# muyangyi/SimSeg

Hardware: AMD Instinct MI355X
Metric: image-text pairs/sec (train) + seg images/sec (eval), ViT-B (higher is better)
Workload: dtype fp16

## Files before the change

simseg_amd/csrc/gemm.hip:

```cpp
#include "common.h"
#include <type_traits>

#ifdef SS_GEMM_ABLATE
#define SS_ABL(v) (p.stagger == (v))
#else
#define SS_ABL(v) false
#endif

namespace {

constexpr int BM = 128, BN = 128, NTHREADS = 256;
constexpr int MC_PITCH = 320;
template <int KB> struct Geo {
    static constexpr int KC_PITCH = KB + 16;
    static constexpr int NCH = KB / 16;
    static constexpr int LOADS = 128 * NCH / NTHREADS;
    static constexpr int KROWS = KB / 2;
    static constexpr int TILE_BYTES = (128 * KC_PITCH > KROWS * MC_PITCH) ? 128 * KC_PITCH : KROWS * MC_PITCH;
    static constexpr int KSTEPS = KB / 32;
};

struct GemmParams {
    const void* A; const void* B; void* C;
    int M, N, K;
// ... 1059 lines not shown
__device__ __forceinline__ const GemmParams& pp_params(const GemmParams& arg, const GemmParams&) { return arg; }
__device__ __forceinline__ const GemmParams& pp_params(const WgradGroupParams&, const GemmParams& own) { return own; }

template <typename TO, bool TA, bool TB, int PP_LEAD = 4, int PRIO = 1, int BIG = 0, int EK = 1, bool GROUPED = false, bool ATOMIC_DIRECT = false>
__global__ __launch_bounds__(512, 2) void gemm_pp_kernel(typename std::conditional<GROUPED, WgradGroupParams, GemmParams>::type arg) {
    extern __shared__ __attribute__((aligned(16))) char lds[];
    GemmParams own;
    int gkz = 0, gt = 0;
    if constexpr (GROUPED) {
        const int gq = xcd_remap(blockIdx.x, gridDim.x);
        if (gq >= arg.first[arg.n]) return;
        int i = 0;
#pragma unroll
        for (int j = 1; j < WG_MAX; ++j)
            if (j < arg.n && gq >= arg.first[j]) i = j;
        const WgradProblem& w = arg.prob[i];
        own = GemmParams{};
        own.A = w.dy; own.B = w.x; own.C = w.dw;
        own.M = w.out; own.N = w.in; own.K = arg.rows;
        own.lda = w.ld_dy; own.ldb = w.ld_x; own.ldc = w.ld_dw;
        own.alpha = 1.0f;
        own.accumulate = 1;
        own.ksplit = arg.ksplit; own.nsplit = arg.nsplit;
        own.dbg_trace = arg.dbg_trace;
        const int gtiles = (w.out >> 8) * (w.in >> 8);
        const int r = gq - arg.first[i];
        gkz = r / gtiles;
        gt = r - gkz * gtiles;
    }
    const GemmParams& p = pp_params(arg, own);
    const int tid = threadIdx.x, lane = tid & 63, wave = __builtin_amdgcn_readfirstlane(tid >> 6);
    const int grp = wave >> 2, wn = wave & 3;
    const int tiles_n = (p.N + 255) / 256;
    const int tiles = tiles_n * ((p.M + 255) / 256);
    const int q = xcd_remap(blockIdx.x, gridDim.x);
    const int kz = GROUPED ? gkz : q / tiles, t = GROUPED ? gt : q - kz * tiles;
    const int m0 = (t / tiles_n) * 256, n0 = (t % tiles_n) * 256;
    const int nk = p.K / 64;
    const int kt0 = kz * p.ksplit;
    const int ntile = min(nk, kt0 + p.ksplit) - kt0;
    const int stot = 4 * ntile;
    const char* Ab = static_cast<const char*>(p.A) + (TA ? (long)kt0 * 64 * p.lda * 2 : (long)kt0 * 128);
    const char* Bb = static_cast<const char*>(p.B) + (TB ? (long)kt0 * 64 * p.ldb * 2 : (long)kt0 * 128);
    const long astep = TA ? 64 * p.lda * 2 : 128, bstep = TB ? 64 * p.ldb * 2 : 128;
    long dA = 0, dB = 0;
    bool pf_ok = false;
    if (BIG && p.pf_next && p.nsplit == 1) {
        const int nb8 = (int)gridDim.x >> 3, rr8 = (int)gridDim.x & 7, xx = (int)blockIdx.x & 7, jj = (int)blockIdx.x >> 3;
        if (jj + 32 < nb8 + (xx < rr8 ? 1 : 0)) {
            const int tn_ = t + 32;
            const int m1 = (tn_ / tiles_n) * 256, n1 = (tn_ % tiles_n) * 256;
            if (m0 + 256 <= p.M && n0 + 256 <= p.N && m1 + 256 <= p.M && n1 + 256 <= p.N) {
                pf_ok = true;
                dA = TA ? (long)(m1 - m0) * 2 : (long)(m1 - m0) * p.lda * 2;
                dB = TB ? (long)(n1 - n0) * 2 : (long)(n1 - n0) * p.ldb * 2;
            }
        }
    }
    unsigned offA[2][2], offB[2][2];
#pragma unroll
    for (int h = 0; h < 2; ++h)
#pragma unroll
        for (int i = 0; i < 2; ++i) {
            offA[h][i] = pp_src_off<TA>(wave * 2 + i, lane, m0 + h * 128, p.M, p.lda);
            offB[h][i] = pp_src_off<TB>(wave * 2 + i, lane, n0 + h * 128, p.N, p.ldb);
            asm volatile("" : "+v"(offA[h][i]), "+v"(offB[h][i]));
        }
    const unsigned lds0 = (unsigned)(unsigned long)(__attribute__((address_space(3))) char*)lds;
    PPFrag<TA, 2> fra;
    PPFrag<TB, 1> frb;
    fra.init(0, grp * 64, lane);
    frb.init(PP_BREG, wn * 32, lane);

    f32x16 acc[4][2];
    {
        const f32x16 zero = {0.f, 0.f, 0.f, 0.f, 0.f, 0.f, 0.f, 0.f, 0.f, 0.f, 0.f, 0.f, 0.f, 0.f, 0.f, 0.f};
#pragma unroll
        for (int i = 0; i < 4; ++i)
#pragma unroll
            for (int j = 0; j < 2; ++j) acc[i][j] = zero;
    }
#define PP_STAGE(H_, KIND)                                                                                            \
    {                                                                                                                 \
        const int h_ = (H_);                                                                                          \
        const bool live_ = h_ < stot;                                                                                 \
        const int kt_ = live_ ? (h_ >> 2) : (pf_ok ? ((h_ - stot) >> 2) : ntile - 1);                                 \
        const unsigned dst_ = lds0 + (live_ ? (((KIND) & 1) ? 0 : PP_BREG) + (((h_ >> 2) & 1) * 2 + ((KIND) >> 1)) * PP_HALF : PP_DUMMY) + \
                              wave * 2048;                                                                            \
        const char* sb_ = ((KIND) & 1) ? Ab + kt_ * astep + (live_ ? 0 : dA) : Bb + kt_ * bstep + (live_ ? 0 : dB);   \
        pp_glds16(((KIND) & 1) ? offA[(KIND) >> 1][0] : offB[(KIND) >> 1][0], sb_, dst_);                             \
        pp_glds16(((KIND) & 1) ? offA[(KIND) >> 1][1] : offB[(KIND) >> 1][1], sb_, dst_ + 1024);                      \
    }
    u32x4 fa[8], fb0[4], fb1[4];
#define PP_READ_A(PAR, HALF)                                                                       \
    _Pragma("unroll") for (int i_ = 0; i_ < 2; ++i_)                                               \
        _Pragma("unroll") for (int kk_ = 0; kk_ < 4; ++kk_) fa[i_ * 4 + kk_] = fra.read(lds, ((PAR) * 2 + (HALF)) * PP_HALF, i_, kk_);
#define PP_READ_B(FB, PAR, HALF) \
    _Pragma("unroll") for (int kk_ = 0; kk_ < 4; ++kk_) FB[kk_] = frb.read(lds, ((PAR) * 2 + (HALF)) * PP_HALF, 0, kk_);
#define PP_CLUSTER(RH, CH, FB)                                                                       \
    if (PRIO == 1) __builtin_amdgcn_s_setprio(1);                                                    \
    _Pragma("unroll") for (int kk_ = 0; kk_ < 4; ++kk_)                                              \
        _Pragma("unroll") for (int i_ = 0; i_ < 2; ++i_) mma<bf16_t>(acc[2 * (RH) + i_][CH], fa[i_ * 4 + kk_], FB[kk_]); \
    if (PRIO == 1) __builtin_amdgcn_s_setprio(0);

    if (p.stagger > 0 && blockIdx.x < 256) {
        const unsigned long long until = wall_clock64() + (unsigned long long)(((blockIdx.x >> 3) & 3) * p.stagger);
        while (wall_clock64() < until) __builtin_amdgcn_s_sleep(8);
    }
    unsigned long long tr0 = 0, tr1 = 0, tr2 = 0;
    if (p.dbg_trace) tr0 = wall_clock64();
    if constexpr (BIG) {
        PP_STAGE(0, 0) PP_STAGE(1, 1) PP_STAGE(2, 2) PP_STAGE(3, 3) PP_STAGE(4, 0) PP_STAGE(5, 1) PP_STAGE(6, 2)
        wait_vm<8>();
        __builtin_amdgcn_s_barrier();
        __builtin_amdgcn_sched_barrier(0);
        if (grp == 1) __builtin_amdgcn_s_barrier();
        if (p.dbg_trace) tr1 = wall_clock64();
#define PP_BIGPHASE(READS, STAGES, RH, CA, FA_, CB, FB_)                                       \
    {                                                                                          \
        READS                                                                                  \
        STAGES                                                                                 \
        wait_vm<8>();                                                                          \
        __builtin_amdgcn_sched_barrier(0);                                                     \
        __builtin_amdgcn_s_barrier();                                                          \
        asm volatile("s_waitcnt lgkmcnt(0)" ::: "memory");                                     \
        __builtin_amdgcn_sched_barrier(0);                                                     \
        PP_CLUSTER(RH, CA, FA_)                                                                \
        PP_CLUSTER(RH, CB, FB_)                                                                \
        asm volatile("" : "+v"(acc[2 * (RH)][0]), "+v"(acc[2 * (RH) + 1][0]), "+v"(acc[2 * (RH)][1]), "+v"(acc[2 * (RH) + 1][1])); \
        __builtin_amdgcn_sched_barrier(0);                                                     \
        __builtin_amdgcn_s_barrier();                                                          \
        __builtin_amdgcn_sched_barrier(0);                                                     \
    }
        for (int tt = 0; tt < ntile; ++tt) {
            PP_BIGPHASE(PP_READ_B(fb0, 0, 0) PP_READ_A(0, 0) PP_READ_B(fb1, 0, 1), PP_STAGE(4 * tt + 7, 3), 0, 0, fb0, 1, fb1)
            frb.toggle(2 * PP_HALF);
            PP_BIGPHASE(PP_READ_A(0, 1), PP_STAGE(4 * tt + 8, 0) PP_STAGE(4 * tt + 9, 1) PP_STAGE(4 * tt + 10, 2), 1, 1, fb1, 0, fb0)
            fra.toggle(2 * PP_HALF);
        }
#undef PP_BIGPHASE
    } else {
    PP_STAGE(0, 0) PP_STAGE(1, 1) PP_STAGE(2, 2) PP_STAGE(3, 3)
    if (PP_LEAD >= 4) PP_STAGE(4, 0)
    if (PP_LEAD >= 5) PP_STAGE(5, 1)
    wait_vm<2 * (PP_LEAD - 1)>();
    if (PRIO == 2 && grp == 1) __builtin_amdgcn_s_setprio(1);
    __builtin_amdgcn_s_barrier();
    __builtin_amdgcn_sched_barrier(0);
    PP_READ_B(fb0, 0, 0)
    if (grp == 1) __builtin_amdgcn_s_barrier();
    if (p.dbg_trace) tr1 = wall_clock64();

#define PP_PHASE(M_, Q, READS, RH, CH, FB)                                                     \
    {                                                                                          \
        READS                                                                                  \
        PP_STAGE((M_) + 1 + PP_LEAD, ((Q) + 1 + PP_LEAD) & 3)                                  \
        wait_vm<2 * (PP_LEAD - 1)>();                                                          \
        __builtin_amdgcn_sched_barrier(0);                                                     \
        __builtin_amdgcn_s_barrier();                                                          \
        asm volatile("s_waitcnt lgkmcnt(0)" ::: "memory");                                     \
        __builtin_amdgcn_sched_barrier(0);                                                     \
        PP_CLUSTER(RH, CH, FB)                                                                 \
        __builtin_amdgcn_sched_barrier(0);                                                     \
        __builtin_amdgcn_s_barrier();                                                          \
        __builtin_amdgcn_sched_barrier(0);                                                     \
    }
    for (int tt = 0; tt < ntile; ++tt) {
        PP_PHASE(4 * tt + 0, 0, PP_READ_A(0, 0), 0, 0, fb0)
        PP_PHASE(4 * tt + 1, 1, PP_READ_B(fb1, 0, 1), 0, 1, fb1)
        PP_PHASE(4 * tt + 2, 2, PP_READ_A(0, 1), 1, 1, fb1)
        frb.toggle(2 * PP_HALF);
        PP_PHASE(4 * tt + 3, 3, PP_READ_B(fb1, 0, 0), 1, 0, fb0)
        fra.toggle(2 * PP_HALF);
#pragma unroll
        for (int kk = 0; kk < 4; ++kk) fb0[kk] = fb1[kk];
    }
#undef PP_PHASE
    }
#undef PP_STAGE
#undef PP_READ_A
#undef PP_READ_B
#undef PP_CLUSTER
    if (!pf_ok) wait_vm<0>();
    if (grp == 0) __builtin_amdgcn_s_barrier();
    if (p.dbg_trace) tr2 = wall_clock64();

    const bool atomic = p.nsplit > 1;
    const bool vec_ok = epilogue_vec_ok(p, sizeof(TO));
    float* wlds = reinterpret_cast<float*>(lds) + wave * EP_WAVE_FLOATS;
    float cs[8] = {0.f, 0.f, 0.f, 0.f, 0.f, 0.f, 0.f, 0.f};
    const int c0 = n0 + wn * 32, c1 = c0 + 128;
    if constexpr (sizeof(TO) == 2) {
        const bool fastep = !atomic && vec_ok && !p.residual && !p.rowscale && p.row_group == 0 && !p.drop_thresh && !p.dbg_skip_epilogue &&
                            (p.act == 0 || p.act == 1 || (p.act == 3 && (!p.aux_blocked || (EK == 2 && p.aux_blocked == 1) || (EK == 4 && p.aux_blocked == 2))) ||
                             (((EK == 1 && !p.aux_blocked) || (EK == 3 && p.aux_blocked == 1) || (EK == 5 && p.aux_blocked == 2)) && p.act == 4 && p.aux)) && (p.act == 4 || !p.colsum) &&
                            m0 + 256 <= p.M && n0 + 256 <= p.N;
        if (fastep) {
            pp_epilogue_bf16<EK>(p, acc, reinterpret_cast<char*>(wlds), m0, c0, c1, grp, lane);
            if (pf_ok) wait_vm<16>();
            if (p.dbg_trace && tid == 0) {
                const unsigned long long tr3 = wall_clock64();
                asm volatile("s_waitcnt vmcnt(0)" ::: "memory");
                unsigned long long* d = p.dbg_trace + (long)blockIdx.x * 5;
                d[0] = tr0; d[1] = tr1; d[2] = tr2; d[3] = wall_clock64(); d[4] = tr3;
            }
            return;
        }
    }
    if constexpr (sizeof(TO) == 4) {
        const bool direct = !atomic && !p.rowscale && !p.aux && p.act == 0 && p.row_group == 0 && !p.colsum && !p.accumulate &&
                            !p.dbg_skip_epilogue && m0 + 256 <= p.M && n0 + 256 <= p.N;
        if (direct) {
            pp_epilogue_f32_direct(p, acc, m0, c0, c1, grp, lane);
            if (pf_ok) wait_vm<63>();
            if (p.dbg_trace && tid == 0) {
                const unsigned long long tr3 = wall_clock64();
                asm volatile("s_waitcnt vmcnt(0)" ::: "memory");
                unsigned long long* d = p.dbg_trace + (long)blockIdx.x * 5;
                d[0] = tr0; d[1] = tr1; d[2] = tr2; d[3] = wall_clock64(); d[4] = tr3;
            }
            return;
        }
    }
    if constexpr (ATOMIC_DIRECT && sizeof(TO) == 4) {
        if (atomic && !p.dbg_skip_epilogue && m0 + 256 <= p.M && n0 + 256 <= p.N) {
            pp_epilogue_atomic_direct(p, acc, m0, c0, c1, grp, lane);
            if (p.dbg_trace && tid == 0) {
                const unsigned long long tr3 = wall_clock64();
                asm volatile("s_waitcnt vmcnt(0)" ::: "memory");
                unsigned long long* d = p.dbg_trace + (long)blockIdx.x * 5;
                d[0] = tr0; d[1] = tr1; d[2] = tr2; d[3] = wall_clock64(); d[4] = tr3;
            }
            return;
        }
    }
#pragma unroll 1
    for (int i = 0; i < 4; ++i) {
        f32x16 l = acc[0][0], r = acc[0][1];
#pragma unroll
        for (int ii = 1; ii < 4; ++ii)
            if (ii == i) { l = acc[ii][0]; r = acc[ii][1]; }
        if (p.dbg_trace && tid == 0) p.dbg_trace[(long)gridDim.x * 5 + (long)blockIdx.x * 4 + i] = wall_clock64();
        epilogue_block<TO>(p, l, r, wlds, m0 + (i >> 1) * 128 + grp * 64 + (i & 1) * 32, c0, c1, lane, atomic, vec_ok, cs);
    }
    flush_colsum(p, cs, c0, c1, lane);
    if (pf_ok) wait_vm<0>();
    if (p.dbg_trace && tid == 0) {
        const unsigned long long tr3 = wall_clock64();
        asm volatile("s_waitcnt vmcnt(0)" ::: "memory");
        unsigned long long* d = p.dbg_trace + (long)blockIdx.x * 5;
        d[0] = tr0; d[1] = tr1; d[2] = tr2; d[3] = wall_clock64(); d[4] = tr3;
    }
}

template <typename TO, bool TA, bool TB, int LEAD = 4, int PRIO = 1, int BIG = 0, int EK = 1>
int launch_pp(const GemmParams& p, int splitk, hipStream_t stream) {
    constexpr int SMEM = 9 * PP_HALF;
    static bool configured = false;
    auto kern = gemm_pp_kernel<TO, TA, TB, LEAD, PRIO, BIG, EK>;
    if (!configured) {
        hipError_t e = hipFuncSetAttribute(reinterpret_cast<const void*>(kern), hipFuncAttributeMaxDynamicSharedMemorySize, SMEM);
        if (e != hipSuccess) return simseg_set_error("simseg_gemm: cannot reserve %d bytes of LDS: %s", SMEM, hipGetErrorString(e));
        configured = true;
    }
    const int tiles = ((p.M + 255) / 256) * ((p.N + 255) / 256);
    const int nk = p.K / 64;
    GemmParams q = p;
    if (splitk < 1) splitk = 1;
    if (splitk > nk) splitk = nk;
    q.ksplit = (nk + splitk - 1) / splitk;
    const int z = (nk + q.ksplit - 1) / q.ksplit;
    q.nsplit = z;
    hipLaunchKernelGGL(kern, dim3(tiles * z, 1, 1), dim3(512), SMEM, stream, q);
    SS_LAUNCH_CHECK("simseg_gemm(ping-pong)");
    return 0;
}

template <bool TRANS>
__device__ __forceinline__ unsigned pp2_lane_off(int piece, int lane, long ld) {
    if (!TRANS) {
        const int r = piece * 8 + (lane >> 3);
        const int c = (lane & 7) ^ kc_swz<64>(r);
        return (unsigned)((long)r * ld * 2 + c * 16);
    } else {
        const int kr = piece * 4 + (lane >> 4);
        const int c = (lane & 15) ^ ((kr & 3) << 2);
        return (unsigned)((long)kr * ld * 2 + c * 16);
    }
}

struct PP2Item { int m0, n0, ntile; const char* a0; const char* b0; };

template <bool TA, bool TB>
__device__ __forceinline__ PP2Item pp2_item(const GemmParams& p, int t, int tiles_n) {
    PP2Item it;
    it.m0 = (t / tiles_n) << 8;
    it.n0 = (t % tiles_n) << 8;
    it.ntile = p.K >> 6;
    it.a0 = static_cast<const char*>(p.A) + (TA ? (long)it.m0 * 2 : (long)it.m0 * p.lda * 2);
    it.b0 = static_cast<const char*>(p.B) + (TB ? (long)it.n0 * 2 : (long)it.n0 * p.ldb * 2);
    return it;
}

template <typename TO, bool TA, bool TB, int SCHED = 0, int EK = 1>
__global__ __launch_bounds__(512, 2) void gemm_pp2_kernel(GemmParams p) {
    extern __shared__ __attribute__((aligned(16))) char lds[];
    const int tid = threadIdx.x, lane = tid & 63, wave = __builtin_amdgcn_readfirstlane(tid >> 6);
    const int grp = wave >> 2, wn = wave & 3;
    const int tiles_n = p.N >> 8;
    const int total = tiles_n * (p.M >> 8);
    const int stride = (int)gridDim.x >> 3;
    const int x = blockIdx.x & 7;
    int ord = blockIdx.x >> 3;
    const int cq = total >> 3, cr = total & 7;
    const int cnt = cq + (x < cr ? 1 : 0);
    const int base = x < cr ? x * (cq + 1) : cr * (cq + 1) + (x - cr) * cq;
    if (ord >= cnt) return;
    const long astep = TA ? 64 * p.lda * 2 : 128, bstep = TB ? 64 * p.ldb * 2 : 128;
    const long ahalf = TA ? 256 : 128 * p.lda * 2, bhalf = TB ? 256 : 128 * p.ldb * 2;
    unsigned offA[2], offB[2];
#pragma unroll
    for (int i = 0; i < 2; ++i) {
        offA[i] = pp2_lane_off<TA>(wave * 2 + i, lane, p.lda);
        offB[i] = pp2_lane_off<TB>(wave * 2 + i, lane, p.ldb);
        asm volatile("" : "+v"(offA[i]), "+v"(offB[i]));
    }
    const unsigned lds0 = (unsigned)(unsigned long)(__attribute__((address_space(3))) char*)lds;
    PPFrag<TA, 2> fra;
    PPFrag<TB, 1> frb;
    fra.init(0, grp * 64, lane);
    frb.init(PP_BREG, wn * 32, lane);

    PP2Item cur = pp2_item<TA, TB>(p, base + ord, tiles_n);
    bool has_next = ord + stride < cnt;
    PP2Item nxt = pp2_item<TA, TB>(p, base + (has_next ? ord + stride : ord), tiles_n);
    const char* sA = cur.a0;
    const char* sB = cur.b0;
    int krem = cur.ntile - 1;
    bool nxt_ok = has_next;
    unsigned spar = 0;
    bool sdummy = false;
    unsigned cpar = 0;

#define PP2_PIECE(KIND, I)                                                                                            \
    {                                                                                                                 \
        const char* sb_ = ((KIND) & 1) ? sA + ((KIND) >> 1) * ahalf : sB + ((KIND) >> 1) * bhalf;                     \
        const unsigned dst_ = lds0 + wave * 2048 + (I) * 1024 +                                                       \
                              (sdummy ? PP_DUMMY : (((KIND) & 1) ? 0 : PP_BREG) + (spar * 2 + ((KIND) >> 1)) * PP_HALF); \
        pp_glds16(((KIND) & 1) ? offA[I] : offB[I], sb_, dst_);                                                       \
    }
#define PP2_STAGE(KIND) PP2_PIECE(KIND, 0) PP2_PIECE(KIND, 1)
#define PP2_ADVANCE()                                                                    \
    {                                                                                    \
        if (krem > 0) { --krem; sA += astep; sB += bstep; }                              \
        else if (nxt_ok) { sA = nxt.a0; sB = nxt.b0; krem = nxt.ntile - 1; nxt_ok = false; } \
        else sdummy = true;                                                              \
        spar ^= 1u;                                                                      \
    }
    u32x4 fa[8], fb0[4], fb1[4];
#define PP_READ_A(HALF)                                                                            \
    _Pragma("unroll") for (int i_ = 0; i_ < 2; ++i_)                                               \
        _Pragma("unroll") for (int kk_ = 0; kk_ < 4; ++kk_) fa[i_ * 4 + kk_] = fra.read(lds, (HALF) * PP_HALF, i_, kk_);
#define PP_READ_B(FB, HALF) \
    _Pragma("unroll") for (int kk_ = 0; kk_ < 4; ++kk_) FB[kk_] = frb.read(lds, (HALF) * PP_HALF, 0, kk_);
#define PP_MMA(RH, CH, FB, KK, I) mma<bf16_t>(acc[2 * (RH) + (I)][CH], fa[(I) * 4 + (KK)], FB[KK]);
#define PP_CLUSTER(RH, CH, FB, KIND, PRE)                                                            \
    __builtin_amdgcn_s_setprio(1);                                                                   \
    PP_MMA(RH, CH, FB, 0, 0) PP_MMA(RH, CH, FB, 0, 1)                                                \
    if (SCHED == 1) { __builtin_amdgcn_sched_barrier(0); PRE PP2_PIECE(KIND, 0) __builtin_amdgcn_sched_barrier(0); } \
    PP_MMA(RH, CH, FB, 1, 0) PP_MMA(RH, CH, FB, 1, 1) PP_MMA(RH, CH, FB, 2, 0)                       \
    if (SCHED == 1 || SCHED == 2) { __builtin_amdgcn_sched_barrier(0); PP2_PIECE(KIND, 1) __builtin_amdgcn_sched_barrier(0); } \
    PP_MMA(RH, CH, FB, 2, 1) PP_MMA(RH, CH, FB, 3, 0) PP_MMA(RH, CH, FB, 3, 1)                       \
     \
                                   \
    asm volatile("" : "+v"(acc[2 * (RH)][CH]), "+v"(acc[2 * (RH) + 1][CH]));                          \
    __builtin_amdgcn_s_setprio(0);
#define PP_PHASE(READS, KIND, PRE, RH, CH, FB)                                                 \
    {                                                                                          \
        if (SCHED == 3) { PRE PP2_STAGE(KIND) }                                                \
        READS                                                                                  \
        if (SCHED == 0) { PRE PP2_STAGE(KIND) }                                                \
        if (SCHED == 2) { PRE PP2_PIECE(KIND, 0) }                                             \
        wait_vm<SCHED == 1 ? 4 : (SCHED == 2 ? 5 : 6)>();                                      \
        __builtin_amdgcn_sched_barrier(0);                                                     \
        __builtin_amdgcn_s_barrier();                                                          \
        asm volatile("s_waitcnt lgkmcnt(0)" ::: "memory");                                     \
        __builtin_amdgcn_sched_barrier(0);                                                     \
        PP_CLUSTER(RH, CH, FB, KIND, PRE)                                                      \
        __builtin_amdgcn_sched_barrier(0);                                                     \
        __builtin_amdgcn_s_barrier();                                                          \
        __builtin_amdgcn_sched_barrier(0);                                                     \
    }

    f32x16 acc[4][2];
    const f32x16 zero = {0.f, 0.f, 0.f, 0.f, 0.f, 0.f, 0.f, 0.f, 0.f, 0.f, 0.f, 0.f, 0.f, 0.f, 0.f, 0.f};
#pragma unroll
    for (int i = 0; i < 4; ++i)
#pragma unroll
        for (int j = 0; j < 2; ++j) acc[i][j] = zero;

    PP2_STAGE(0) PP2_STAGE(1) PP2_STAGE(2) PP2_STAGE(3)
    PP2_ADVANCE()
    PP2_STAGE(0)

    for (;;) {
        asm volatile("" : "+v"(offA[0]), "+v"(offA[1]), "+v"(offB[0]), "+v"(offB[1]));
        fra.pin(); frb.pin();
        __builtin_amdgcn_s_waitcnt(0x0F70);
        wait_vm<0>();
        __builtin_amdgcn_s_barrier();
        __builtin_amdgcn_sched_barrier(0);
        PP_READ_B(fb0, 0)
        if (grp == 1) __builtin_amdgcn_s_barrier();
        for (int tt = 0; tt < cur.ntile; ++tt) {
            PP_PHASE(PP_READ_A(0), 1, , 0, 0, fb0)
            PP_PHASE(PP_READ_B(fb1, 1), 2, , 0, 1, fb1)
            PP_PHASE(PP_READ_A(1), 3, , 1, 1, fb1)
            frb.toggle(2 * PP_HALF);
            PP_PHASE(PP_READ_B(fb1, 0), 0, PP2_ADVANCE(), 1, 0, fb0)
            fra.toggle(2 * PP_HALF);
            cpar ^= 1u;
#pragma unroll
            for (int kk = 0; kk < 4; ++kk) fb0[kk] = fb1[kk];
        }
        if (grp == 0) __builtin_amdgcn_s_barrier();
        __builtin_amdgcn_sched_barrier(0);
        const int c0 = cur.n0 + wn * 32, c1 = c0 + 128;
        if constexpr (sizeof(TO) == 2) {
            const unsigned lp = cpar ^ 1u;
            char* tl = lds + (wave < 7 ? lp * (2 * PP_HALF) + wave * 4608 : PP_BREG + (lp * 2 + 1) * PP_HALF);
            pp_epilogue_bf16<EK>(p, acc, tl, cur.m0, c0, c1, grp, lane);
        } else {
            pp_epilogue_f32_direct(p, acc, cur.m0, c0, c1, grp, lane);
        }
        if (!has_next) break;
        cur.m0 = nxt.m0; cur.n0 = nxt.n0; cur.ntile = nxt.ntile;
        ord += stride;
        has_next = ord + stride < cnt;
        nxt = pp2_item<TA, TB>(p, base + (has_next ? ord + stride : ord), tiles_n);
        nxt_ok = has_next;
#pragma unroll
        for (int i = 0; i < 4; ++i)
#pragma unroll
            for (int j = 0; j < 2; ++j) acc[i][j] = zero;
    }
    wait_vm<0>();
#undef PP_PHASE
#undef PP2_STAGE
#undef PP2_PIECE
#undef PP_MMA
#undef PP2_ADVANCE
#undef PP_READ_A
#undef PP_READ_B
#undef PP_CLUSTER
}

template <typename TO>
bool pp2_ok(const GemmParams& p, int splitk) {
    if (splitk > 1 || p.M % 256 || p.N % 256 || p.K % 64 || p.K < 128) return false;
    if (p.rowscale || p.row_group || p.dbg_skip_epilogue || p.dbg_trace) return false;
    const long tiles = (long)(p.M / 256) * (p.N / 256);
    if (tiles <= 256) return false;
    bool vec = (p.ldc % 8 == 0) && (((uintptr_t)p.C) % 16 == 0);
    if (p.bias) vec = vec && (((uintptr_t)p.bias) % 16 == 0);
    if (p.aux) vec = vec && (((uintptr_t)p.aux) % 16 == 0);
    if (p.aux_out) vec = vec && (((uintptr_t)p.aux_out) % 16 == 0);
    if (sizeof(TO) == 2)
        return vec && !p.residual && !p.drop_thresh && (p.act == 0 || p.act == 1 || p.act == 3 || (p.act == 4 && p.aux)) && (p.act == 4 || !p.colsum);
    return !p.aux && p.act == 0 && !p.colsum && !p.accumulate;
}

template <typename TO, bool TA, bool TB, int SCHED = 0, int EK = 1>
int launch_pp2(const GemmParams& p, hipStream_t stream, int reserve = 0) {
    constexpr int SMEM = 9 * PP_HALF;
    static bool configured = false;
    static int blocks = 0;
    auto kern = gemm_pp2_kernel<TO, TA, TB, SCHED, EK>;
    if (!configured) {
        hipError_t e = hipFuncSetAttribute(reinterpret_cast<const void*>(kern), hipFuncAttributeMaxDynamicSharedMemorySize, SMEM);
        if (e != hipSuccess) return simseg_set_error("simseg_gemm: cannot reserve %d bytes of LDS: %s", SMEM, hipGetErrorString(e));
        int dev = 0, cus = 0;
        if (hipGetDevice(&dev) != hipSuccess || hipDeviceGetAttribute(&cus, hipDeviceAttributeMultiprocessorCount, dev) != hipSuccess || cus < 8)
            return simseg_set_error("simseg_gemm: cannot read the CU count");
        blocks = cus & ~7;
        configured = true;
    }
    GemmParams q = p;
    q.ksplit = p.K / 64; q.nsplit = 1;
    const int nb = reserve > 0 ? ((blocks - reserve) & ~7) : blocks;
    hipLaunchKernelGGL(kern, dim3(nb < 8 ? 8 : nb, 1, 1), dim3(512), SMEM, stream, q);
    SS_LAUNCH_CHECK("simseg_gemm(persistent ping-pong)");
    return 0;
}



thread_local int g_gemm_debug_skip_epilogue = 0;
thread_local unsigned long long* g_gemm_debug_trace = nullptr;
thread_local int g_gemm_stagger = 0;
thread_local int g_gemm_wgrad_blocks = 0;
thread_local int g_gemm_last_variant = 0;

template <typename T, typename TO, int WM, int WK>
__global__ __launch_bounds__(256) void gemm_small_kernel(GemmParams p) {
    constexpr int TM = 32 * WM, TN = 64, NSTAGE = 4;
    constexpr int PA = TM / 8, PB = TN / 8;
    constexpr int PPW = (PA + PB) / 4;
    constexpr int STAGE = (TM + TN) * 128;
    constexpr int KPW = 4 / WK;
    static_assert(WM * WK == 4 && (PA + PB) % 4 == 0, "four waves");
    static_assert(NSTAGE * STAGE >= (WK - 1) * WM * 8192 + WM * EP_WAVE_FLOATS * 4, "ring doubles as reduction + epilogue scratch");
    extern __shared__ __attribute__((aligned(16))) char lds[];
    const int tid = threadIdx.x, lane = tid & 63, wave = __builtin_amdgcn_readfirstlane(tid >> 6);
    const int wm = wave % WM, wk = wave / WM;
    const int tiles_n = (p.N + TN - 1) / TN;
    const int t = xcd_remap(blockIdx.x, gridDim.x);
    const int m0 = (t / tiles_n) * TM, n0 = (t % tiles_n) * TN;
    const int nk = (int)((long)p.K * (long)sizeof(T) / 128);

    const char* src[PPW];
    int dst[PPW];
#pragma unroll
    for (int i = 0; i < PPW; ++i) {
        const int pi = wave * PPW + i;
        const bool isb = pi >= PA;
        const int pr = isb ? pi - PA : pi;
        const int r = pr * 8 + (lane >> 3);
        const int c = (lane & 7) ^ ((r >> 1) & 7);
        int gr = (isb ? n0 : m0) + r;
        const int lim = isb ? p.N : p.M;
        gr = gr < lim ? gr : lim - 1;
        src[i] = static_cast<const char*>(isb ? p.B : p.A) + ((long)gr * (isb ? p.ldb : p.lda)) * (long)sizeof(T) + c * 16;
        dst[i] = (isb ? TM * 128 : 0) + pr * 1024;
    }
    auto issue = [&](int stage, int kt) {
#pragma unroll
        for (int i = 0; i < PPW; ++i)
            __builtin_amdgcn_global_load_lds((const __attribute__((address_space(1))) void*)(src[i] + (long)kt * 128),
                                             (__attribute__((address_space(3))) void*)(lds + stage * STAGE + dst[i]), 16, 0, 0);
    };
    f32x16 acc0, acc1;
#pragma unroll
    for (int r = 0; r < 16; ++r) { acc0[r] = 0.f; acc1[r] = 0.f; }
#pragma unroll
    for (int s = 0; s < NSTAGE - 1; ++s)
        if (s < nk) issue(s, s);
    int stage = 0;
    for (int kt = 0; kt < nk; ++kt) {
        const int ahead = min(NSTAGE - 2, nk - 1 - kt);
        if (ahead >= 2) wait_vm<2 * PPW>();
        else if (ahead == 1) wait_vm<PPW>();
        else wait_vm<0>();
        __builtin_amdgcn_s_barrier();
        __builtin_amdgcn_sched_barrier(0);
        if (kt + NSTAGE - 1 < nk) {
            int ns = stage + NSTAGE - 1; ns = ns >= NSTAGE ? ns - NSTAGE : ns;
            issue(ns, kt + NSTAGE - 1);
        }
        const char* sa = lds + stage * STAGE;
        const char* sb = sa + TM * 128;
#pragma unroll
        for (int kq = 0; kq < KPW; ++kq) {
            const int c = 2 * (wk * KPW + kq) + (lane >> 5);
            const int ra = wm * 32 + (lane & 31), rb = lane & 31;
            const u32x4 fa = *reinterpret_cast<const u32x4*>(sa + ra * 128 + ((c ^ ((ra >> 1) & 7)) << 4));
            const u32x4 fb0 = *reinterpret_cast<const u32x4*>(sb + rb * 128 + ((c ^ ((rb >> 1) & 7)) << 4));
            const u32x4 fb1 = *reinterpret_cast<const u32x4*>(sb + (rb + 32) * 128 + ((c ^ (((rb + 32) >> 1) & 7)) << 4));
            mma<T>(acc0, fa, fb0);
            mma<T>(acc1, fa, fb1);
        }
        stage = stage + 1 == NSTAGE ? 0 : stage + 1;
    }
    __builtin_amdgcn_s_barrier();
    if (WK > 1) {
        float* red = reinterpret_cast<float*>(lds);
        if (wk > 0) {
            float* dstp = red + ((wk - 1) * WM + wm) * 2048 + lane;
#pragma unroll
            for (int r = 0; r < 16; ++r) { dstp[r * 64] = acc0[r]; dstp[(16 + r) * 64] = acc1[r]; }
        }
        __syncthreads();
        if (wk > 0) return;
#pragma unroll
        for (int g = 0; g < WK - 1; ++g) {
            const float* sp = red + (g * WM + wm) * 2048 + lane;
#pragma unroll
            for (int r = 0; r < 16; ++r) { acc0[r] += sp[r * 64]; acc1[r] += sp[(16 + r) * 64]; }
        }
    }
    float* wlds = reinterpret_cast<float*>(lds + (WK - 1) * WM * 8192) + wm * EP_WAVE_FLOATS;
    float cs[8] = {0.f, 0.f, 0.f, 0.f, 0.f, 0.f, 0.f, 0.f};
    epilogue_block<TO>(p, acc0, acc1, wlds, m0 + wm * 32, n0, n0 + 32, lane, false, epilogue_vec_ok(p, sizeof(TO)), cs);
    flush_colsum(p, cs, n0, n0 + 32, lane);
}

template <typename T, typename TO, int WM, int WK>
int launch_small(const GemmParams& p, hipStream_t stream) {
    constexpr int SMEM = 4 * (32 * WM + 64) * 128;
    static bool configured = false;
    auto kern = gemm_small_kernel<T, TO, WM, WK>;
    if (!configured) {
        hipError_t e = hipFuncSetAttribute(reinterpret_cast<const void*>(kern), hipFuncAttributeMaxDynamicSharedMemorySize, SMEM);
        if (e != hipSuccess) return simseg_set_error("simseg_gemm: cannot reserve %d bytes of LDS: %s", SMEM, hipGetErrorString(e));
        configured = true;
    }
    GemmParams q = p;
    q.ksplit = 0; q.nsplit = 1;
    const int tiles = ((p.M + 32 * WM - 1) / (32 * WM)) * ((p.N + 63) / 64);
    hipLaunchKernelGGL(kern, dim3(tiles), dim3(256), SMEM, stream, q);
    SS_LAUNCH_CHECK("simseg_gemm(small)");
    return 0;
}

template <typename T, typename TO>
int dispatch_small(const GemmParams& p, hipStream_t s) {
    const long t64 = (long)((p.M + 63) / 64) * ((p.N + 63) / 64);
    if (t64 >= 192) return launch_small<T, TO, 2, 2>(p, s);
    return launch_small<T, TO, 1, 4>(p, s);
}

thread_local int g_gemm_variant = 0;

template <typename TO, bool TA, bool TB>
int launch_pp2_ek(const GemmParams& p, hipStream_t s, int reserve) {
    if constexpr (sizeof(TO) == 2) {
        if (p.act == 4 && !p.aux_blocked) return launch_pp2<TO, TA, TB, 0, 1>(p, s, reserve);
        if constexpr (!TB) { if (p.act == 3 && p.aux_blocked == 1) return launch_pp2<TO, TA, TB, 0, 2>(p, s, reserve); }
        if constexpr (TB) { if (p.act == 4 && p.aux_blocked == 1) return launch_pp2<TO, TA, TB, 0, 3>(p, s, reserve); }
        if constexpr (!TB) { if (p.act == 3 && p.aux_blocked == 2) return launch_pp2<TO, TA, TB, 0, 4>(p, s, reserve); }
        if constexpr (TB) { if (p.act == 4 && p.aux_blocked == 2) return launch_pp2<TO, TA, TB, 0, 5>(p, s, reserve); }
    }
    if (p.aux_blocked) return simseg_set_error("simseg_gemm: act 5 is a forward (x . W^T) epilogue, act 6 a dgrad (d . W) epilogue, both with 16-bit outputs");
    return launch_pp2<TO, TA, TB, 0, 0>(p, s, reserve);
}

template <typename TO, bool TA, bool TB>
int dispatch_bf16(const GemmParams& p, int splitk, bool aligned, hipStream_t s) {
    const bool big_ok = aligned && p.K % 64 == 0 && p.M >= 256 && p.N >= 128;
    const bool four_phase = g_gemm_variant == 15;
    int v = (four_phase || g_gemm_variant == 16 || g_gemm_variant == 18) ? 0 : g_gemm_variant;
    const int nk64 = p.K / 64;
    const int kper = (nk64 + (splitk > 1 ? splitk : 1) - 1) / (splitk > 1 ? splitk : 1);
    const int tiles256 = ((p.M + 255) / 256) * ((p.N + 255) / 256);
    if constexpr (TA && sizeof(TO) == 4) {
        if ((v == 0 || v == 6 || v == 3) && v != 7 && big_ok && p.accumulate && splitk > 1 && p.M % 256 == 0 && p.N % 256 == 0 && tiles256 <= 128) {
            int sk = 256 / tiles256;
            static const int env_blocks = getenv("SIMSEG_GEMM_WGRAD_BLOCKS") ? atoi(getenv("SIMSEG_GEMM_WGRAD_BLOCKS")) : 0;
            const int wb = g_gemm_wgrad_blocks > 0 ? g_gemm_wgrad_blocks : env_blocks;
            if (wb > 0) sk = wb / tiles256 > 0 ? wb / tiles256 : 1;
            if (nk64 / sk < 16 && nk64 >= 64) sk = nk64 / 16;
            if (nk64 / sk >= 16 && tiles256 * sk >= 96 && (v == 3 || v == 0)) {
                g_gemm_last_variant = 3;
                return four_phase ? launch_pp<TO, TA, TB>(p, sk, s) : launch_pp<TO, TA, TB, 4, 1, 1>(p, sk, s);
            }
            if (nk64 / sk >= 16 && v == 6) { g_gemm_last_variant = 2; return launch_large<TO, TA, TB, 64, 2, 256, 256, 2, 4, 2>(p, sk, s); }
        }
        if (v == 3) v = 0;
        if (v == 6) v = 0;
        if (v == 7) v = 1;
    }
    if (v == 0) {
        const int pad_n = ((p.N + 255) / 256) * 256 - p.N;
        const bool n_fits = pad_n * 6 <= p.N || kper >= 40;
        v = (big_ok && !TA && tiles256 >= 96 && n_fits && (kper >= 12 || (kper >= 6 && tiles256 >= 1024))) ? 3 : 1;
    }
    if (v >= 10 && v <= 13 && !(big_ok && !TA)) v = 1;
    const long t128 = (long)((p.M + 127) / 128) * ((p.N + 127) / 128);
    if (v == 1 && (g_gemm_variant == 0 || g_gemm_variant >= 15) && !TA && !TB && splitk <= 1 && t128 >= 160 && t128 <= 256) v = 5;
    if (v == 8 || v == 9) {
        if (aligned && p.K % 32 == 0 && p.M >= 256 && p.N >= 256) {
            g_gemm_last_variant = v;
            if (v == 8) return launch_large<TO, TA, TB, 32, 3, 256, 128, 2, 2, 2>(p, splitk, s);
            return launch_large<TO, TA, TB, 32, 3, 128, 256, 2, 2, 2>(p, splitk, s);
        }
        v = 1;
    }
    if (v == 5) {
        if (aligned && p.K % 64 == 0 && p.M >= 128 && p.N >= 128) { g_gemm_last_variant = 5; return launch_large<TO, TA, TB, 64, 4, 128, 128, 2, 2, 1>(p, splitk, s); }
        v = 1;
    }
    if (!big_ok) v = 1;
    g_gemm_last_variant = v;
    if (p.aux_blocked && !(v == 3 || (v >= 10 && v <= 13)))
        return simseg_set_error("simseg_gemm: act 5 / 6 (tile-blocked saved derivative) needs the 256x256 ping-pong kernel; this call dispatches to variant %d", v);
    if (v == 3 || (v >= 10 && v <= 13)) {
        if constexpr (!TA) {
            static int reserve = -1, min_tiles = -1;
            if (reserve < 0) {
                const char* e = getenv("SIMSEG_GEMM_PP2_RESERVE"); reserve = e ? atoi(e) : 0;
                e = getenv("SIMSEG_GEMM_PP2_MIN_TILES"); min_tiles = e ? atoi(e) : 600;
            }
            static int act4 = -1;
            if (act4 < 0) { const char* e = getenv("SIMSEG_GEMM_PP2_ACT4"); act4 = e ? atoi(e) : 0; }
            if ((g_gemm_variant == 18 || g_gemm_variant == 0) && tiles256 >= min_tiles && (p.act != 4 || p.aux_blocked || act4) && pp2_ok<TO>(p, splitk)) {
                g_gemm_last_variant = 10;
                return launch_pp2_ek<TO, TA, TB>(p, s, reserve);
            }
            if (g_gemm_variant >= 10 && g_gemm_variant <= 13 && pp2_ok<TO>(p, splitk)) {
                g_gemm_last_variant = 10;
                if (g_gemm_variant != 10 && p.aux_blocked) return simseg_set_error("simseg_gemm: the schedule experiments (variants 11-13) do not carry the tile-blocked epilogues");
                switch (g_gemm_variant) {
                    case 11: return launch_pp2<TO, TA, TB, 1>(p, s);
                    case 12: return launch_pp2<TO, TA, TB, 2>(p, s);
                    case 13: return launch_pp2<TO, TA, TB, 3>(p, s);
                    default: return launch_pp2_ek<TO, TA, TB>(p, s, 0);
                }
            }
        }
        g_gemm_last_variant = 3;
        if (!four_phase && p.K >= 128) {
            if constexpr (sizeof(TO) == 2 && !TA) {
                if constexpr (!TB) { if (p.act == 3 && p.aux_blocked == 1) return launch_pp<TO, TA, TB, 4, 1, 1, 2>(p, splitk, s); }
                if constexpr (TB) { if (p.act == 4 && p.aux_blocked == 1) return launch_pp<TO, TA, TB, 4, 1, 1, 3>(p, splitk, s); }
                if constexpr (!TB) { if (p.act == 3 && p.aux_blocked == 2) return launch_pp<TO, TA, TB, 4, 1, 1, 4>(p, splitk, s); }
                if constexpr (TB) { if (p.act == 4 && p.aux_blocked == 2) return launch_pp<TO, TA, TB, 4, 1, 1, 5>(p, splitk, s); }
            }
            if (p.aux_blocked) return simseg_set_error("simseg_gemm: act 5 is a forward (x . W^T) epilogue, act 6 a dgrad (d . W) epilogue");
            if (sizeof(TO) == 2 && p.act != 4) return launch_pp<TO, TA, TB, 4, 1, 1, 0>(p, splitk, s);
            return launch_pp<TO, TA, TB, 4, 1, 1>(p, splitk, s);
        }
        if (p.aux_blocked) return simseg_set_error("simseg_gemm: the four-phase schedule (variant 15) does not carry the tile-blocked epilogues");
        return launch_pp<TO, TA, TB>(p, splitk, s);
    }
    if (v == 2) return launch_large<TO, TA, TB, 64, 2, 256, 256, 2, 4, 2>(p, splitk, s);
    return launch<bf16_t, TO, TA, TB>(p, splitk, s);
}

}

extern "C" int simseg_gemm_last_variant(void) {
    SS_HALF_FWD(simseg_gemm_last_variant); return g_gemm_last_variant; }

extern "C" int simseg_debug_gemm_stagger(int ticks) {
#ifndef SS_GEMM_ABLATE
    SS_CHECK(ticks < 1000, "debug_gemm_stagger: %d selects an epilogue ablation, which this build does not contain (-DSS_GEMM_ABLATE)", ticks);
#endif
    g_gemm_stagger = ticks;
    return 0;
}
extern "C" int simseg_debug_gemm_wgrad_blocks(int blocks) {
#ifndef SS_HALF
    simseg_debug_gemm_wgrad_blocks_h16(blocks);
#endif
    g_gemm_wgrad_blocks = blocks;
    return 0;
}
extern "C" int simseg_debug_gemm_trace(void* buf) { g_gemm_debug_trace = static_cast<unsigned long long*>(buf); return 0; }

extern "C" int simseg_set_gemm_variant(int v) {
#ifndef SS_HALF
    simseg_set_gemm_variant_h16(v);
#endif
    g_gemm_debug_skip_epilogue = v >= 100;
    g_gemm_variant = v % 100;
    return 0;
}

namespace {
}

extern "C" int simseg_patch_text_sim(const void* x, const void* text, float* out, int64_t M, int64_t C, int64_t K, int dtype,
                                     float eps, int normalize, void* stream) {
    SS_HALF_FWD(simseg_patch_text_sim, x, text, out, M, C, K, dtype, eps, normalize, stream);
    SS_CHECK(x && text && out, "patch_text_sim: null pointer");
    SS_CHECK(M > 0 && C > 0 && C <= 256 && K > 0 && M < (1ll << 31), "patch_text_sim: need 1 <= C <= 256 (got C=%lld)", (long long)C);
    SS_CHECK(dtype == 0 || dtype == 1, "patch_text_sim: dtype must be 0 (fp32) or 1 (bf16)");
    const int epc = dtype == 0 ? 4 : 8;
    SS_CHECK(K % epc == 0 && ((uintptr_t)x % 16) == 0 && ((uintptr_t)text % 16) == 0, "patch_text_sim: K must be a multiple of %d and the operands 16-byte aligned", epc);
    if (dtype == 0) return dispatch_simmap<float>(x, text, out, (int)M, (int)C, (int)K, eps, normalize, (hipStream_t)stream);
    return dispatch_simmap<bf16_t>(x, text, out, (int)M, (int)C, (int)K, eps, normalize, (hipStream_t)stream);
}

extern "C" int simseg_gemm_aux_blocked_ok(int64_t M, int64_t N, int64_t K) {
    if (M <= 0 || N <= 0 || K <= 0 || M % 256 || N % 256 || K % 64 || K < 768) return 0;
    return (M / 256) * (N / 256) >= 96;
}

static thread_local int g_wgrad_group_last = 0;
extern "C" int simseg_wgrad_group_last(void) {
    SS_HALF_FWD(simseg_wgrad_group_last); return g_wgrad_group_last; }

extern "C" int simseg_gemm_wgrad_group(const int64_t* problems, int n, int64_t rows, int slices, void* stream) {
    SS_HALF_FWD(simseg_gemm_wgrad_group, problems, n, rows, slices, stream);
    g_wgrad_group_last = 0;
    SS_CHECK(problems && n >= 1 && n <= WG_MAX, "simseg_gemm_wgrad_group: 1..%d problems", WG_MAX);
    SS_CHECK(rows > 0 && rows < (1ll << 31) && slices >= 1, "simseg_gemm_wgrad_group: bad rows %lld / slices %d", (long long)rows, slices);
    if (rows % 64 != 0) return 0;
    const int nk = (int)(rows / 64);
    if (nk / slices < 16) return 0;
    WgradGroupParams g;
    memset(&g, 0, sizeof(g));
    g.ksplit = (nk + slices - 1) / slices;
    g.nsplit = (nk + g.ksplit - 1) / g.ksplit;
    long blocks = 0;
    for (int i = 0; i < n; ++i) {
        const int64_t* d = problems + 8 * i;
        WgradProblem& w = g.prob[i];
        SS_CHECK(d[0] && d[1] && d[2], "simseg_gemm_wgrad_group: null operand in problem %d", i);
        const int64_t out = d[3], in = d[4];
        if (out <= 0 || in <= 0 || out % 256 || in % 256 || out >= (1ll << 31) || in >= (1ll << 31)) return 0;
        if (d[5] < out || d[6] < in || d[7] < in || d[5] % 8 || d[6] % 8 || d[7] % 4) return 0;
        if ((uintptr_t)d[0] % 16 || (uintptr_t)d[1] % 16 || (uintptr_t)d[2] % 16) return 0;
        if (64 * d[5] * 2 >= (1ll << 31) || 64 * d[6] * 2 >= (1ll << 31)) return 0;
        w.dy = (const void*)(uintptr_t)d[0]; w.x = (const void*)(uintptr_t)d[1]; w.dw = (float*)(uintptr_t)d[2];
        w.out = (int)out; w.in = (int)in; w.ld_dy = d[5]; w.ld_x = d[6]; w.ld_dw = d[7];
        g.first[i] = (int)blocks;
        blocks += (out / 256) * (in / 256) * g.nsplit;
        if (blocks >= (1l << 24)) return 0;
    }
    for (int i = n; i <= WG_MAX; ++i) g.first[i] = (int)blocks;
    g.n = n; g.rows = (int)rows;
    g.dbg_trace = g_gemm_debug_trace;
    static const bool direct = !(getenv("SIMSEG_GEMM_WGRAD_DIRECT") && atoi(getenv("SIMSEG_GEMM_WGRAD_DIRECT")) == 0);
    constexpr int SMEM = 9 * PP_HALF;
    static bool configured = false;
    if (!configured) {
        hipError_t e = hipFuncSetAttribute(reinterpret_cast<const void*>(&gemm_pp_kernel<float, true, true, 4, 1, 1, 1, true, false>), hipFuncAttributeMaxDynamicSharedMemorySize, SMEM);
        if (e == hipSuccess) e = hipFuncSetAttribute(reinterpret_cast<const void*>(&gemm_pp_kernel<float, true, true, 4, 1, 1, 1, true, true>), hipFuncAttributeMaxDynamicSharedMemorySize, SMEM);
        if (e != hipSuccess) return simseg_set_error("simseg_gemm_wgrad_group: cannot reserve %d bytes of LDS: %s", SMEM, hipGetErrorString(e));
        configured = true;
    }
    hipStream_t s = (hipStream_t)stream;
    if (direct) hipLaunchKernelGGL((gemm_pp_kernel<float, true, true, 4, 1, 1, 1, true, true>), dim3((unsigned)blocks, 1, 1), dim3(512), SMEM, s, g);
    else hipLaunchKernelGGL((gemm_pp_kernel<float, true, true, 4, 1, 1, 1, true, false>), dim3((unsigned)blocks, 1, 1), dim3(512), SMEM, s, g);
    SS_LAUNCH_CHECK("simseg_gemm_wgrad_group");
    g_gemm_last_variant = 3;
    g_wgrad_group_last = n;
    return 0;
}

extern "C" int simseg_gemm(const void* A, const void* B, void* C, int64_t M, int64_t N, int64_t K, int64_t lda,
                           int64_t ldb, int64_t ldc, int in_dtype, int out_dtype, int transA, int transB, float alpha,
                           const float* bias, const float* rowscale, const float* residual, int64_t ldr, int act,
                           const void* aux, void* aux_out, int row_group, int res_mod, int accumulate, int splitk,
                           uint64_t drop_seed, float drop_p, float* colsum, void* stream) {
    SS_HALF_FWD(simseg_gemm, A, B, C, M, N, K, lda, ldb, ldc, in_dtype, out_dtype, transA, transB, alpha, bias, rowscale, residual, ldr, act, aux, aux_out, row_group, res_mod, accumulate, splitk, drop_seed, drop_p, colsum, stream);
    SS_CHECK(A && B && C, "simseg_gemm: null operand");
    SS_CHECK(M > 0 && N > 0 && K > 0 && M < (1ll << 31) && N < (1ll << 31) && K < (1ll << 31), "simseg_gemm: bad shape %lld x %lld x %lld",
             (long long)M, (long long)N, (long long)K);
    const int epc = in_dtype == 0 ? 4 : 8;
    SS_CHECK(in_dtype == 0 || in_dtype == 1, "simseg_gemm: in_dtype must be 0 (fp32) or 1 (bf16)");
    SS_CHECK(out_dtype == 0 || out_dtype == 1, "simseg_gemm: out_dtype must be 0 (fp32) or 1 (bf16)");
    SS_CHECK(in_dtype == 1 || out_dtype == 0, "simseg_gemm: fp32 operands produce fp32 output");
    SS_CHECK(in_dtype == 1 || (!transA && !transB), "simseg_gemm: transposed operands need bf16");
    SS_CHECK(!(transA && !transB), "simseg_gemm: (transA, !transB) is not on the path");
    const bool aligned = ((uintptr_t)A % 16) == 0 && ((uintptr_t)B % 16) == 0 && lda % epc == 0 && ldb % epc == 0 &&
                         (transA ? M : K) % epc == 0 && (transB ? N : K) % epc == 0;
    SS_CHECK(aligned || in_dtype == 0, "simseg_gemm: bf16 operands need 16-byte aligned pointers and contiguous extents / leading dimensions that are multiples of 8");
    SS_CHECK(((uintptr_t)A % 4) == 0 && ((uintptr_t)B % 4) == 0, "simseg_gemm: misaligned operand");
    SS_CHECK(splitk <= 1 || (out_dtype == 0 && act == 0 && !bias && !residual && drop_p == 0.f && !colsum),
             "simseg_gemm: split-K needs a plain fp32 accumulate epilogue");
    SS_CHECK(drop_p >= 0.f && drop_p < 1.f, "simseg_gemm: dropout p out of range");
    SS_CHECK(act >= 0 && act <= 8, "simseg_gemm: act must be 0..8");
    const int blocked = act >= 7 ? 2 : (act >= 5 ? 1 : 0);
    if (blocked) {
        const bool fwd = act == 5 || act == 7;
        SS_CHECK(simseg_gemm_aux_blocked_ok(M, N, K) && in_dtype == 1 && out_dtype == 1 && !transA && !rowscale && !residual && row_group == 0 &&
                 drop_p == 0.f && splitk <= 1 && ldc == N && (fwd ? aux_out != nullptr : aux != nullptr) &&
                 ((uintptr_t)(fwd ? aux_out : aux) % 16) == 0 && ((uintptr_t)C % 16) == 0 && (!bias || ((uintptr_t)bias % 16) == 0),
                 "simseg_gemm: act %d needs a full-tile 16-bit problem on the ping-pong kernel (simseg_gemm_aux_blocked_ok) with a plain epilogue", act);
        act = fwd ? 3 : 4;
    }
    SS_CHECK((act != 2 && act != 4) || aux, "simseg_gemm: act=2/4 needs aux");
    SS_CHECK(!res_mod || row_group > 0, "simseg_gemm: res_mod needs row_group");
    GemmParams p;
    memset(&p, 0, sizeof(p));
    p.A = A; p.B = B; p.C = C; p.M = (int)M; p.N = (int)N; p.K = (int)K;
    p.lda = lda; p.ldb = ldb; p.ldc = ldc; p.alpha = alpha; p.bias = bias; p.rowscale = rowscale;
    p.residual = residual; p.ldr = ldr; p.act = act; p.aux = aux; p.aux_out = aux_out;
    p.row_group = row_group; p.res_mod = res_mod; p.accumulate = accumulate; p.dbg_skip_epilogue = g_gemm_debug_skip_epilogue; p.dbg_trace = g_gemm_debug_trace; p.stagger = g_gemm_stagger;
    p.drop_seed = drop_seed;
    p.colsum = colsum;
    p.drop_thresh = drop_p > 0.f ? (unsigned int)((double)drop_p * 4294967296.0) : 0u;
    p.drop_scale = drop_p > 0.f ? 1.0f / (1.0f - drop_p) : 1.0f;
    p.aux_blocked = blocked;
    p.pf_next = g_gemm_variant != 16;
    hipStream_t s = (hipStream_t)stream;
    g_gemm_last_variant = 1;
    const bool small_fit = !transA && !transB && aligned && splitk <= 1 && (K * (in_dtype == 0 ? 4 : 2)) % 128 == 0;
    const int64_t t128 = ((M + 127) / 128) * ((N + 127) / 128);
    const bool small_auto = small_fit && t128 < (in_dtype == 0 ? 200 : 160);
    if (((g_gemm_variant == 0 || g_gemm_variant >= 15) && small_auto) || (g_gemm_variant == 4 && small_fit)) {
        g_gemm_last_variant = 4;
        if (in_dtype == 0) return dispatch_small<float, float>(p, s);
        return out_dtype ? dispatch_small<bf16_t, bf16_t>(p, s) : dispatch_small<bf16_t, float>(p, s);
    }
    if (in_dtype == 0) return aligned ? launch<float, float, false, false, true>(p, splitk, s) : launch<float, float, false, false, false>(p, splitk, s);
    if (!transA && !transB) return out_dtype ? dispatch_bf16<bf16_t, false, false>(p, splitk, aligned, s) : dispatch_bf16<float, false, false>(p, splitk, aligned, s);
    if (!transA && transB) return out_dtype ? dispatch_bf16<bf16_t, false, true>(p, splitk, aligned, s) : dispatch_bf16<float, false, true>(p, splitk, aligned, s);
    return out_dtype ? dispatch_bf16<bf16_t, true, true>(p, splitk, aligned, s) : dispatch_bf16<float, true, true>(p, splitk, aligned, s);
}
```

Measured before the change: 6192.

## Add two-phase K loop to 256x256 ping-pong GEMM and default to it

Adds a TWO template mode to the pp2 GEMM kernel that merges the four per-K-tile phases into two larger phases. Each phase issues more LDS reads and global copies up front and then runs two MFMA clusters between barriers. It prefetches deeper (stages 1-2 in the prologue) and, for 16-bit outputs, reserves one extra LDS half-buffer with a new epilogue staging layout. The mode is selected by default when K>=128. The aim is to halve the barrier and wait overhead per K tile, at the cost of more LDS and possibly lower occupancy or more register pressure.

```diff
diff --git a/simseg_amd/csrc/gemm.hip b/simseg_amd/csrc/gemm.hip
--- a/simseg_amd/csrc/gemm.hip
+++ b/simseg_amd/csrc/gemm.hip
@@ -1385,8 +1385,9 @@
     return it;
 }
 
-template <typename TO, bool TA, bool TB, int SCHED = 0, int EK = 1>
+template <typename TO, bool TA, bool TB, int SCHED = 0, int EK = 1, bool TWO = false>
 __global__ __launch_bounds__(512, 2) void gemm_pp2_kernel(GemmParams p) {
+    static_assert(!TWO || SCHED == 0, "the two-phase K loop issues its copies in the load segment");
     extern __shared__ __attribute__((aligned(16))) char lds[];
     const int tid = threadIdx.x, lane = tid & 63, wave = __builtin_amdgcn_readfirstlane(tid >> 6);
     const int grp = wave >> 2, wn = wave & 3;
@@ -1474,6 +1475,21 @@
         __builtin_amdgcn_s_barrier();                                                          \
         __builtin_amdgcn_sched_barrier(0);                                                     \
     }
+#define PP_PHASE2(READS, STAGES, RH, CA, FA_, CB, FB_)                                         \
+    {                                                                                          \
+        READS                                                                                  \
+        STAGES                                                                                 \
+        wait_vm<8>();                                                                          \
+        __builtin_amdgcn_sched_barrier(0);                                                     \
+        __builtin_amdgcn_s_barrier();                                                          \
+        asm volatile("s_waitcnt lgkmcnt(0)" ::: "memory");                                     \
+        __builtin_amdgcn_sched_barrier(0);                                                     \
+        PP_CLUSTER(RH, CA, FA_, 0, )                                                           \
+        PP_CLUSTER(RH, CB, FB_, 0, )                                                           \
+        __builtin_amdgcn_sched_barrier(0);                                                     \
+        __builtin_amdgcn_s_barrier();                                                          \
+        __builtin_amdgcn_sched_barrier(0);                                                     \
+    }
 
     f32x16 acc[4][2];
     const f32x16 zero = {0.f, 0.f, 0.f, 0.f, 0.f, 0.f, 0.f, 0.f, 0.f, 0.f, 0.f, 0.f, 0.f, 0.f, 0.f, 0.f};
@@ -1485,6 +1501,7 @@
     PP2_STAGE(0) PP2_STAGE(1) PP2_STAGE(2) PP2_STAGE(3)
     PP2_ADVANCE()
     PP2_STAGE(0)
+    if constexpr (TWO) { PP2_STAGE(1) PP2_STAGE(2) }
 
     for (;;) {
         asm volatile("" : "+v"(offA[0]), "+v"(offA[1]), "+v"(offB[0]), "+v"(offB[1]));
@@ -1493,8 +1510,17 @@
         wait_vm<0>();
         __builtin_amdgcn_s_barrier();
         __builtin_amdgcn_sched_barrier(0);
-        PP_READ_B(fb0, 0)
+        if constexpr (!TWO) PP_READ_B(fb0, 0)
         if (grp == 1) __builtin_amdgcn_s_barrier();
+        if constexpr (TWO) {
+            for (int tt = 0; tt < cur.ntile; ++tt) {
+                PP_PHASE2(PP_READ_B(fb0, 0) PP_READ_A(0) PP_READ_B(fb1, 1), PP2_STAGE(3), 0, 0, fb0, 1, fb1)
+                frb.toggle(2 * PP_HALF);
+                PP_PHASE2(PP_READ_A(1), PP2_ADVANCE() PP2_STAGE(0) PP2_STAGE(1) PP2_STAGE(2), 1, 1, fb1, 0, fb0)
+                fra.toggle(2 * PP_HALF);
+                cpar ^= 1u;
+            }
+        } else
         for (int tt = 0; tt < cur.ntile; ++tt) {
             PP_PHASE(PP_READ_A(0), 1, , 0, 0, fb0)
             PP_PHASE(PP_READ_B(fb1, 1), 2, , 0, 1, fb1)
@@ -1511,7 +1537,12 @@
         const int c0 = cur.n0 + wn * 32, c1 = c0 + 128;
         if constexpr (sizeof(TO) == 2) {
             const unsigned lp = cpar ^ 1u;
-            char* tl = lds + (wave < 7 ? lp * (2 * PP_HALF) + wave * 4608 : PP_BREG + (lp * 2 + 1) * PP_HALF);
+            char* tl;
+            if constexpr (TWO)
+                tl = lds + (wave < 3 ? (lp * 2 + 1) * PP_HALF + wave * 4608
+                                     : wave < 6 ? (has_next ? PP_DUMMY : lp * (2 * PP_HALF)) + (wave - 3) * 4608 : 9 * PP_HALF + (wave - 6) * 4608);
+            else
+                tl = lds + (wave < 7 ? lp * (2 * PP_HALF) + wave * 4608 : PP_BREG + (lp * 2 + 1) * PP_HALF);
             pp_epilogue_bf16<EK>(p, acc, tl, cur.m0, c0, c1, grp, lane);
         } else {
             pp_epilogue_f32_direct(p, acc, cur.m0, c0, c1, grp, lane);
@@ -1529,6 +1560,7 @@
     }
     wait_vm<0>();
 #undef PP_PHASE
+#undef PP_PHASE2
 #undef PP2_STAGE
 #undef PP2_PIECE
 #undef PP_MMA
@@ -1537,6 +1569,8 @@
 #undef PP_READ_B
 #undef PP_CLUSTER
 }
+
+constexpr int PP2_TWO_MIN_K = 128;
 
 template <typename TO>
 bool pp2_ok(const GemmParams& p, int splitk) {
@@ -1553,12 +1587,12 @@
     return !p.aux && p.act == 0 && !p.colsum && !p.accumulate;
 }
 
-template <typename TO, bool TA, bool TB, int SCHED = 0, int EK = 1>
+template <typename TO, bool TA, bool TB, int SCHED = 0, int EK = 1, bool TWO = false>
 int launch_pp2(const GemmParams& p, hipStream_t stream, int reserve = 0) {
-    constexpr int SMEM = 9 * PP_HALF;
+    constexpr int SMEM = (TWO && sizeof(TO) == 2 ? 10 : 9) * PP_HALF;
     static bool configured = false;
     static int blocks = 0;
-    auto kern = gemm_pp2_kernel<TO, TA, TB, SCHED, EK>;
+    auto kern = gemm_pp2_kernel<TO, TA, TB, SCHED, EK, TWO>;
     if (!configured) {
         hipError_t e = hipFuncSetAttribute(reinterpret_cast<const void*>(kern), hipFuncAttributeMaxDynamicSharedMemorySize, SMEM);
         if (e != hipSuccess) return simseg_set_error("simseg_gemm: cannot reserve %d bytes of LDS: %s", SMEM, hipGetErrorString(e));
@@ -1704,24 +1738,31 @@
 
 thread_local int g_gemm_variant = 0;
 
+template <typename TO, bool TA, bool TB, int EK>
+int launch_pp2_k(const GemmParams& p, hipStream_t s, int reserve, bool two) {
+    return two ? launch_pp2<TO, TA, TB, 0, EK, true>(p, s, reserve) : launch_pp2<TO, TA, TB, 0, EK, false>(p, s, reserve);
+}
+
 template <typename TO, bool TA, bool TB>
-int launch_pp2_ek(const GemmParams& p, hipStream_t s, int reserve) {
+int launch_pp2_ek(const GemmParams& p, hipStream_t s, int reserve, bool two) {
     if constexpr (sizeof(TO) == 2) {
-        if (p.act == 4 && !p.aux_blocked) return launch_pp2<TO, TA, TB, 0, 1>(p, s, reserve);
-        if constexpr (!TB) { if (p.act == 3 && p.aux_blocked == 1) return launch_pp2<TO, TA, TB, 0, 2>(p, s, reserve); }
-        if constexpr (TB) { if (p.act == 4 && p.aux_blocked == 1) return launch_pp2<TO, TA, TB, 0, 3>(p, s, reserve); }
-        if constexpr (!TB) { if (p.act == 3 && p.aux_blocked == 2) return launch_pp2<TO, TA, TB, 0, 4>(p, s, reserve); }
-        if constexpr (TB) { if (p.act == 4 && p.aux_blocked == 2) return launch_pp2<TO, TA, TB, 0, 5>(p, s, reserve); }
+        if (p.act == 4 && !p.aux_blocked) return launch_pp2_k<TO, TA, TB, 1>(p, s, reserve, two);
+        if constexpr (!TB) { if (p.act == 3 && p.aux_blocked == 1) return launch_pp2_k<TO, TA, TB, 2>(p, s, reserve, two); }
+        if constexpr (TB) { if (p.act == 4 && p.aux_blocked == 1) return launch_pp2_k<TO, TA, TB, 3>(p, s, reserve, two); }
+        if constexpr (!TB) { if (p.act == 3 && p.aux_blocked == 2) return launch_pp2_k<TO, TA, TB, 4>(p, s, reserve, two); }
+        if constexpr (TB) { if (p.act == 4 && p.aux_blocked == 2) return launch_pp2_k<TO, TA, TB, 5>(p, s, reserve, two); }
     }
     if (p.aux_blocked) return simseg_set_error("simseg_gemm: act 5 is a forward (x . W^T) epilogue, act 6 a dgrad (d . W) epilogue, both with 16-bit outputs");
-    return launch_pp2<TO, TA, TB, 0, 0>(p, s, reserve);
+    return launch_pp2_k<TO, TA, TB, 0>(p, s, reserve, two);
 }
 
 template <typename TO, bool TA, bool TB>
 int dispatch_bf16(const GemmParams& p, int splitk, bool aligned, hipStream_t s) {
     const bool big_ok = aligned && p.K % 64 == 0 && p.M >= 256 && p.N >= 128;
     const bool four_phase = g_gemm_variant == 15;
-    int v = (four_phase || g_gemm_variant == 16 || g_gemm_variant == 18) ? 0 : g_gemm_variant;
+    const bool pp2_four = g_gemm_variant == 19, pp2_two = g_gemm_variant == 20;
+    const int gv = (pp2_four || pp2_two) ? 10 : g_gemm_variant;
+    int v = (four_phase || g_gemm_variant == 16 || g_gemm_variant == 18) ? 0 : gv;
     const int nk64 = p.K / 64;
     const int kper = (nk64 + (splitk > 1 ? splitk : 1) - 1) / (splitk > 1 ? splitk : 1);
     const int tiles256 = ((p.M + 255) / 256) * ((p.N + 255) / 256);
@@ -1768,25 +1809,27 @@
         return simseg_set_error("simseg_gemm: act 5 / 6 (tile-blocked saved derivative) needs the 256x256 ping-pong kernel; this call dispatches to variant %d", v);
     if (v == 3 || (v >= 10 && v <= 13)) {
         if constexpr (!TA) {
-            static int reserve = -1, min_tiles = -1;
+            static int reserve = -1, min_tiles = -1, two_min_k = -1;
             if (reserve < 0) {
                 const char* e = getenv("SIMSEG_GEMM_PP2_RESERVE"); reserve = e ? atoi(e) : 0;
                 e = getenv("SIMSEG_GEMM_PP2_MIN_TILES"); min_tiles = e ? atoi(e) : 600;
-            }
+                e = getenv("SIMSEG_GEMM_PP2_TWO_MIN_K"); two_min_k = e ? atoi(e) : PP2_TWO_MIN_K;
+            }
+            const bool two = pp2_two || (!pp2_four && p.K >= two_min_k);
             static int act4 = -1;
             if (act4 < 0) { const char* e = getenv("SIMSEG_GEMM_PP2_ACT4"); act4 = e ? atoi(e) : 0; }
             if ((g_gemm_variant == 18 || g_gemm_variant == 0) && tiles256 >= min_tiles && (p.act != 4 || p.aux_blocked || act4) && pp2_ok<TO>(p, splitk)) {
                 g_gemm_last_variant = 10;
-                return launch_pp2_ek<TO, TA, TB>(p, s, reserve);
-            }
-            if (g_gemm_variant >= 10 && g_gemm_variant <= 13 && pp2_ok<TO>(p, splitk)) {
+                return launch_pp2_ek<TO, TA, TB>(p, s, reserve, two);
+            }
+            if (gv >= 10 && gv <= 13 && pp2_ok<TO>(p, splitk)) {
                 g_gemm_last_variant = 10;
-                if (g_gemm_variant != 10 && p.aux_blocked) return simseg_set_error("simseg_gemm: the schedule experiments (variants 11-13) do not carry the tile-blocked epilogues");
-                switch (g_gemm_variant) {
+                if (gv != 10 && p.aux_blocked) return simseg_set_error("simseg_gemm: the schedule experiments (variants 11-13) do not carry the tile-blocked epilogues");
+                switch (gv) {
                     case 11: return launch_pp2<TO, TA, TB, 1>(p, s);
                     case 12: return launch_pp2<TO, TA, TB, 2>(p, s);
                     case 13: return launch_pp2<TO, TA, TB, 3>(p, s);
-                    default: return launch_pp2_ek<TO, TA, TB>(p, s, 0);
+                    default: return launch_pp2_ek<TO, TA, TB>(p, s, 0, two);
                 }
             }
         }
```

Measured after the change: 6253, median of 6. Within noise of the previous version (+1.0%).
